# limix/CellRegMap

Measured on AMD Instinct MI355X. Metric: variant-tests/sec (interaction test), higher is better.
Workload: dtype f64

## Files before the change

cellregmap_amd/csrc/assemble.hip:

```cpp
#include "assemble.h"
#include "wave_ops.h"

namespace crm {

namespace {

__global__ __launch_bounds__(256) void woodbury_kernel(AssembleArgs a, const double* __restrict__ Gw, int KT,
                                                       double* __restrict__ Gext) {
    extern __shared__ double wsm[];
    const int k1 = a.wb_k1, KW = KT + k1, k0 = a.k0, c = a.c;
    const int b = blockIdx.x, tid = threadIdx.x;
    const NullFitOut fit = a.fit[b];
    const double g = fit.v0 * a.rho[fit.rho_index].rho;
    const double inv = 1.0 / fit.v1;
    const double* __restrict__ G = Gw + (long)b * KW * KW;
    double* __restrict__ out = Gext + (long)b * KT * KT;
    if (!(g > 0.0)) {
        for (int e = tid; e < KT * KT; e += 256) out[e] = G[(long)(e / KT) * KW + e % KT];
        return;
    }
    double* ME = wsm;
    double* Cm = ME + KT * k1;
    double* Z = Cm + k1 * k1;
    const long pos = a.sorted_pos[b];
    for (int e = tid; e < KT * k1; e += 256) {
        const int u = e / k1, f = e - u * k1;
        double plain;
        if (u < k0) plain = pos >= 0 ? a.wb_E1X[(long)f * a.wb_ldE1X + pos * k0 + u] : 0.0;
        else if (u < k0 + c) plain = a.wb_E1yW[(long)f * a.wb_ldE1yW + 1 + (u - k0)];
        else if (u == k0 + c) plain = a.wb_E1g[(long)f * a.wb_ldE1g + b];
        else plain = a.wb_E1yW[(long)f * a.wb_ldE1yW];
        ME[e] = (u < k0 && pos < 0) ? 0.0 : (plain - G[(long)u * KW + KT + f]) * inv;
    }
    for (int e = tid; e < k1 * k1; e += 256) {
        const int i = e / k1, j = e - i * k1;
        Cm[e] = (i == j ? 1.0 : 0.0) + g * (a.wb_EE[e] - G[(long)(KT + i) * KW + KT + j]) * inv;
    }
    __syncthreads();
    for (int j = 0; j < k1; j++) {
        if (tid == 0) Cm[j * k1 + j] = sqrt(Cm[j * k1 + j]);
        __syncthreads();
        const double l = Cm[j * k1 + j];
        for (int i = j + 1 + tid; i < k1; i += 256) Cm[i * k1 + j] /= l;
        __syncthreads();
        for (int e = tid; e < (k1 - j - 1) * (k1 - j - 1); e += 256) {
            const int i = j + 1 + e / (k1 - j - 1), q = j + 1 + e % (k1 - j - 1);
            if (q <= i) Cm[i * k1 + q] -= Cm[i * k1 + j] * Cm[q * k1 + j];
        }
        __syncthreads();
    }
    for (int u = tid; u < KT; u += 256) {
        for (int i = 0; i < k1; i++) {
            double s = ME[u * k1 + i];
            for (int q = 0; q < i; q++) s -= Cm[i * k1 + q] * Z[q * KT + u];
            Z[i * KT + u] = s / Cm[i * k1 + i];
        }
        for (int i = k1 - 1; i >= 0; i--) {
            double s = Z[i * KT + u];
            for (int q = i + 1; q < k1; q++) s -= Cm[q * k1 + i] * Z[q * KT + u];
            Z[i * KT + u] = s / Cm[i * k1 + i];
        }
    }
    __syncthreads();
    const double scale = fit.v1 * g;
    for (int e = tid; e < KT * KT; e += 256) {
        const int u = e / KT, v = e - u * KT;
        double s = 0.0;
        for (int f = 0; f < k1; f++) s += ME[u * k1 + f] * Z[f * KT + v];
        out[e] = G[(long)u * KW + v] + scale * s;
    }
}

__global__ __launch_bounds__(256) void woodbury_yty_kernel(AssembleArgs a, const double* __restrict__ Gw, int KT,
                                                           double* __restrict__ Gext) {
    extern __shared__ double wsm[];
    const int k1 = a.wb_k1, KW = KT + k1, k0 = a.k0, c = a.c;
    const int NR = k1 + KT, LD = NR | 1;
    const int b = blockIdx.x, tid = threadIdx.x;
    const int lane = tid & 63, wave = __builtin_amdgcn_readfirstlane(tid >> 6);
    const NullFitOut fit = a.fit[b];
    const double g = fit.v0 * a.rho[fit.rho_index].rho;
    const double inv = 1.0 / fit.v1;
    const double* __restrict__ G = Gw + (long)b * KW * KW;
    double* __restrict__ out = Gext + (long)b * KT * KT;
    if (!(g > 0.0)) {
        for (int e = tid; e < KT * KT; e += 256) out[e] = G[(long)(e / KT) * KW + e % KT];
        return;
    }
    double* AT = wsm;
    const long pos = a.sorted_pos[b];
    for (int e = tid; e < KT * k1; e += 256) {
        const int u = e / k1, f = e - u * k1;
        double plain;
        if (u < k0) plain = pos >= 0 ? a.wb_E1X[(long)f * a.wb_ldE1X + pos * k0 + u] : 0.0;
        else if (u < k0 + c) plain = a.wb_E1yW[(long)f * a.wb_ldE1yW + 1 + (u - k0)];
        else if (u == k0 + c) plain = a.wb_E1g[(long)f * a.wb_ldE1g + b];
        else plain = a.wb_E1yW[(long)f * a.wb_ldE1yW];
        AT[f * LD + k1 + u] = (u < k0 && pos < 0) ? 0.0 : (plain - G[(long)u * KW + KT + f]) * inv;
    }
    for (int e = tid; e < k1 * k1; e += 256) {
        const int i = e / k1, j = e - i * k1;
        if (j <= i) AT[j * LD + i] = (i == j ? 1.0 : 0.0) + g * (a.wb_EE[e] - G[(long)(KT + i) * KW + KT + j]) * inv;
    }
    __syncthreads();
    if (wave == 0) {
        const double l = sqrt(AT[0]);
        for (int R = lane; R < NR; R += 64) AT[R] = R == 0 ? l : AT[R] / l;
    }
    __syncthreads();
    for (int j = 0; j + 1 < k1; j++) {
        const double* colj = AT + j * LD;
        const double lnext = wave == 0 ? sqrt(fma(-colj[j + 1], colj[j + 1], AT[(j + 1) * LD + j + 1])) : 0.0;
        for (int R = ((j + 1) & ~63) + lane; R < NR; R += 64) {
            const double aR = R > j ? colj[R] : 0.0;
            for (int q0 = j + 1 + wave; q0 < k1; q0 += 16) {
                double lq[4], cv[4];
#pragma unroll
                for (int m = 0; m < 4; m++) {
                    const int q = q0 + 4 * m;
                    const bool on = q < k1 && R >= q;
                    lq[m] = on ? colj[q] : 0.0;
                    cv[m] = on ? AT[q * LD + R] : 0.0;
                }
#pragma unroll
                for (int m = 0; m < 4; m++) {
                    const int q = q0 + 4 * m;
                    if (!(q < k1 && R >= q)) continue;
                    double v = fma(-aR, lq[m], cv[m]);
                    if (q == j + 1) v = R == q ? lnext : v / lnext;
                    AT[q * LD + R] = v;
                }
            }
        }
        __syncthreads();
    }
    const int ts = (KT + 15) / 16, l15 = lane & 15, l4 = lane >> 4;
    const double scale = fit.v1 * g;
    const double* __restrict__ Y = AT + k1;
    int t = 0;
    for (int ti = 0; ti < ts; ti++)
        for (int tj = ti; tj < ts; tj++, t++) {
            if ((t & 3) != wave) continue;
            const int u = 16 * ti + l15, v = 16 * tj + l15;
            v4d acc = (v4d){0.0, 0.0, 0.0, 0.0};
            for (int f0 = 0; f0 < k1; f0 += 4) {
                const int f = f0 + l4;
                const double fa = (f < k1 && u < KT) ? Y[f * LD + u] : 0.0;
                const double fb = (f < k1 && v < KT) ? Y[f * LD + v] : 0.0;
                acc = __builtin_amdgcn_mfma_f64_16x16x4f64(fa, fb, acc, 0, 0, 0);
            }
#pragma unroll
            for (int reg = 0; reg < 4; reg++) {
                const int row = 16 * ti + l4 + 4 * reg;
                if (row < KT && v < KT && v >= row) {
                    const double s = scale * acc[reg];
                    out[(long)row * KT + v] = G[(long)row * KW + v] + s;
                    if (v != row) out[(long)v * KT + row] = G[(long)v * KW + row] + s;
                }
            }
        }
}

constexpr int PMAX = CRM_MAX_COV_XWIDE + 1;

__global__ __launch_bounds__(128) void finalize_kernel(AssembleArgs a, const double* __restrict__ Gext,
                                                        int KT, double* __restrict__ rows, int sym) {
    extern __shared__ double fsm[];
    __shared__ int ok_flag, keep_flag;
    __shared__ double rescale;
    const int Pd = a.c + 1;
    double* Lm = fsm;
    double* xky = Lm + Pd * Pd;
    double* uvec = xky + Pd;
    double* vv = uvec + a.k0;
    double* ww = vv + Pd;
    double* dkxm = rows ? rows + (size_t)blockIdx.x * 2 * a.k0 * Pd : ww + Pd;
    double* solm = dkxm + a.k0 * Pd;
#define L(i, j) Lm[(i) * Pd + (j)]
#define dkx(j, i) dkxm[(j) * Pd + (i)]
#define sol(j, i) solm[(j) * Pd + (i)]
    const int b = blockIdx.x;
    const NullFitOut fit = a.fit[b];
    const int k0 = a.k0, c = a.c;
    const int P = c + 1;
    const double v1 = fit.v1;
    const double inv = 1.0 / v1;
    const double* __restrict__ Ge = Gext + (long)b * KT * KT;
    const int tid = threadIdx.x;
    auto plain_xx = [&](int i, int j) -> double {
        if (i > j) { int t = i; i = j; j = t; }
        if (j < c) return a.WW[i * c + j];
        if (i < c) return a.gW[(long)b * a.ld_gW + i];
        return a.gg[b];
    };
    auto plain_xy = [&](int i) -> double { return i < c ? a.Wy[i] : a.gy[b]; };

    if (tid == 0) {
        bool ok = true;
        for (int i = 0; i < P; i++) {
            for (int j = 0; j <= i; j++)
                L(i, j) = (plain_xx(i, j) - Ge[(long)(k0 + i) * KT + (k0 + j)]) * inv;
            xky[i] = (plain_xy(i) - Ge[(long)(k0 + i) * KT + (k0 + c + 1)]) * inv;
        }
        bool keep = true;
        for (int j = 0; j < P && ok; j++) {
            double d = L(j, j);
            for (int k = 0; k < j; k++) d -= L(j, k) * L(j, k);
            if (!(d > 0.0)) {
                if (j == c) keep = false;
                else ok = false;
                break;
            }
            const double l = sqrt(d);
            L(j, j) = l;
            for (int i = j + 1; i < P; i++) {
                double s = L(i, j);
                for (int k = 0; k < j; k++) s -= L(i, k) * L(j, k);
                L(i, j) = s / l;
            }
        }
        if (ok && keep) {
            double nrm2 = 1.0;
            {
                for (int i = c - 1; i >= 0; i--) {
                    double sacc = L(c, i);
                    for (int k = i + 1; k < c; k++) sacc -= L(k, i) * vv[k];
                    vv[i] = sacc / L(i, i);
                }
                for (int j = 0; j < c; j++) {
                    const double t = vv[j] + (a.coef ? a.coef[(long)j * a.ld_coef + b] : 0.0);
                    nrm2 += t * t;
                }
            }
            const double lam_min = L(c, c) * L(c, c) / nrm2;
            for (int i = 0; i < P; i++) vv[i] = 1.0;
            double lam_max = 0.0;
            for (int it = 0; it < 12; it++) {
                const double vl = vv[c];
                for (int j = 0; j < c; j++) ww[j] = vv[j] + (a.coef ? a.coef[(long)j * a.ld_coef + b] : 0.0) * vl;
                ww[c] = vl;
                for (int i = 0; i < P; i++) {
                    double sacc = 0.0;
                    for (int k = i; k < P; k++) sacc += L(k, i) * ww[k];
                    vv[i] = sacc;
                }
                for (int i = P - 1; i >= 0; i--) {
                    double sacc = 0.0;
                    for (int k = 0; k <= i; k++) sacc += L(i, k) * vv[k];
                    ww[i] = sacc;
                }
                double last = ww[c];
                for (int j = 0; j < c; j++) last += (a.coef ? a.coef[(long)j * a.ld_coef + b] : 0.0) * ww[j];
                double n2 = last * last;
                for (int j = 0; j < c; j++) n2 += ww[j] * ww[j];
                lam_max = sqrt(n2);
                if (!(lam_max > 0.0)) break;
                for (int j = 0; j < c; j++) vv[j] = ww[j] / lam_max;
                vv[c] = last / lam_max;
            }
            if (lam_min <= 2.220446049250313e-16 * (double)P * lam_max) keep = false;
        }
        if (!keep) {
            for (int j = 0; j < c; j++) L(c, j) = 0.0;
            L(c, c) = 1.0;
            xky[c] = 0.0;
        }
        keep_flag = keep ? 1 : 0;
        rescale = 1.0;
        if (ok) {
            for (int i = 0; i < P; i++) {
                double s = xky[i];
                for (int k = 0; k < i; k++) s -= L(i, k) * xky[k];
                xky[i] = s / L(i, i);
            }
            if (fit.scale < 0.0) {
                double r = (a.yy - Ge[(long)(k0 + c + 1) * KT + (k0 + c + 1)]) * inv;
                const int used = c + ((fit.use_g && keep) ? 1 : 0);
                for (int i = 0; i < used; i++) r -= xky[i] * xky[i];
                const double df = (double)a.n - (double)(c + (fit.use_g ? 1 : 0));
                rescale = 1.0 / fmax(r / df, 1.4901161193847656e-08);
            }
            for (int i = P - 1; i >= 0; i--) {
                double s = xky[i];
                for (int k = i + 1; k < P; k++) s -= L(k, i) * xky[k];
                xky[i] = s / L(i, i);
            }
        }
        ok_flag = ok ? 1 : 0;
    }
    __syncthreads();
    const bool ok = ok_flag != 0;
    const bool keep_g = keep_flag != 0;
    for (int j = tid; j < k0; j += blockDim.x) {
        double row[PMAX];
        for (int i = 0; i < P; i++) {
            double plain;
            if (i < c) plain = a.Z1[(long)b * a.ldZ1 + (long)(1 + i) * k0 + j];
            else plain = a.Z2[(long)b * a.ldZ2 + j];
            double v = (plain - Ge[(long)j * KT + (k0 + i)]) * inv;
            if (i == c && !keep_g) v = 0.0;
            row[i] = v;
            dkx(j, i) = v;
        }
        for (int i = 0; i < P; i++) {
            double s = row[i];
            for (int k = 0; k < i; k++) s -= L(i, k) * row[k];
            row[i] = s / L(i, i);
        }
        for (int i = P - 1; i >= 0; i--) {
            double s = row[i];
            for (int k = i + 1; k < P; k++) s -= L(k, i) * row[k];
            row[i] = s / L(i, i);
        }
        for (int i = 0; i < P; i++) sol(j, i) = row[i];
        const double dky = (a.Z1[(long)b * a.ldZ1 + j] - Ge[(long)j * KT + (k0 + c + 1)]) * inv;
        double u = dky;
        for (int i = 0; i < P; i++) u -= dkx(j, i) * xky[i];
        uvec[j] = u * rescale;
    }
    __syncthreads();
    if (tid == 0) {
        double q = 0.0;
        for (int j = 0; j < k0; j++) q += uvec[j] * uvec[j];
        a.Q[b] = ok ? 0.5 * q : NAN;
    }
    double* __restrict__ F = a.F + (long)b * k0 * k0;
    for (int e = tid; e < k0 * k0; e += blockDim.x) {
        const int j = e / k0, jp = e - j * k0;
        const int lo = j < jp ? j : jp, hi = j < jp ? jp : j;
        const long pidx = (long)lo * k0 - (long)lo * (lo - 1) / 2 + (hi - lo);
        const int ja = sym ? lo : j, jb = sym ? hi : jp;
        double v = (a.Z3[(long)b * a.ldZ3 + pidx] - Ge[(long)ja * KT + jb]) * inv;
        for (int i = 0; i < P; i++) v -= dkx(ja, i) * sol(jb, i);
        F[e] = ok ? 0.5 * v * rescale : NAN;
    }
}
#undef L
#undef dkx
#undef sol

}

size_t woodbury_lds_bytes(int KT, int k1) { return sizeof(double) * ((size_t)2 * KT * k1 + (size_t)k1 * k1); }

size_t assemble_rows_scratch_doubles(int variants, int k0, int c) {
    const size_t P = (size_t)c + 1;
    const size_t lds = sizeof(double) * (P * P + 3 * P + k0 + 2 * (size_t)k0 * P);
    return lds > 150 * 1024 ? (size_t)variants * 2 * k0 * P : 0;
}

int launch_assemble(hipStream_t st, const AssembleArgs& a, int variants, double* Gext, double* fin_rows,
                    long* dma_launches) {
    if (variants <= 0) return CRM_OK;
    const int KT0 = a.k0 + a.c + 2;
    const int KT = KT0 + (a.wb_k1 > 0 ? a.wb_k1 : 0);
    double* const Gfin = Gext;
    if (a.wb_k1 > 0) {
        if (KT > CRM_MAX_GRAM_ROWS || woodbury_lds_bytes(KT0, a.wb_k1) > 150 * 1024 || !a.wb_Gw) {
            set_error("assemble: unrelated-donor form with %d + %d rows outside its supported range", KT0, a.wb_k1);
            return CRM_ERR_INTERNAL;
        }
        Gext = a.wb_Gw;
    }
    const int P = a.c + 1;
    const size_t fin_small = sizeof(double) * ((size_t)P * P + 3 * P + a.k0);
    size_t fin_lds = fin_small + sizeof(double) * 2 * (size_t)a.k0 * P;
    const bool rows_global = fin_lds > 150 * 1024;
    if (rows_global) fin_lds = fin_small;
    if (a.k0 > CRM_MAX_K0 || a.c > CRM_MAX_COV_XWIDE || KT > CRM_MAX_GRAM_ROWS || (rows_global && !fin_rows)) {
        set_error("assemble: k0=%d, c=%d outside the supported range (k0 <= %d, c <= %d, k0 + c + 2 <= %d)", a.k0, a.c,
                  CRM_MAX_K0, CRM_MAX_COV_XWIDE, CRM_MAX_GRAM_ROWS);
        return CRM_ERR_UNSUPPORTED;
    }
    const bool gram_done = a.wb_k1 > 0 && a.wb_gram_done != 0;
    bool dma = gram_done;
    if (!gram_done) CRM_TRY(launch_gram_ext(st, a, variants, Gext, KT, &dma));
    if (dma && dma_launches) ++*dma_launches;
    const bool yty = a.wb_k1 > 0 && form("woodbury_ytY", 1) != 0;
    if (a.wb_k1 > 0) {
        const size_t lds = yty ? sizeof(double) * a.wb_k1 * (size_t)((KT0 + a.wb_k1) | 1) : woodbury_lds_bytes(KT0, a.wb_k1);
        CRM_HIP(yty ? launch_with_lds(woodbury_yty_kernel, dim3(variants), dim3(256), lds, st, lds > 60 * 1024, a, a.wb_Gw, KT0, Gfin)
                    : launch_with_lds(woodbury_kernel, dim3(variants), dim3(256), lds, st, lds > 60 * 1024, a, a.wb_Gw, KT0, Gfin));
    }
    CRM_HIP(launch_with_lds(finalize_kernel, dim3(variants), dim3(128), fin_lds, st, fin_lds > 60 * 1024, a, Gfin, KT0,
                            rows_global ? fin_rows : nullptr, yty ? 1 : 0));
    return CRM_OK;
}

}
```

Measured before the change: 85530.

## Add single-wave row-oriented Cholesky path to Woodbury ytY kernel

```diff
diff --git a/cellregmap_amd/csrc/assemble.hip b/cellregmap_amd/csrc/assemble.hip
--- a/cellregmap_amd/csrc/assemble.hip
+++ b/cellregmap_amd/csrc/assemble.hip
@@ -71,6 +71,17 @@
     }
 }
 
+constexpr int CB = 4;
+
+__device__ __forceinline__ void rows_take_left(double (&v)[CB], const double* own, const double* lq, int LD, int q0) {
+    for (int j = 0; j < q0; j++) {
+        const double aj = own[j * LD];
+#pragma unroll
+        for (int m = 0; m < CB; m++) v[m] = fma(-aj, lq[j * LD + m], v[m]);
+    }
+}
+
+template <int ROWS>
 __global__ __launch_bounds__(256) void woodbury_yty_kernel(AssembleArgs a, const double* __restrict__ Gw, int KT,
                                                            double* __restrict__ Gext) {
     extern __shared__ double wsm[];
@@ -89,50 +100,135 @@
     }
     double* AT = wsm;
     const long pos = a.sorted_pos[b];
-    for (int e = tid; e < KT * k1; e += 256) {
-        const int u = e / k1, f = e - u * k1;
-        double plain;
-        if (u < k0) plain = pos >= 0 ? a.wb_E1X[(long)f * a.wb_ldE1X + pos * k0 + u] : 0.0;
-        else if (u < k0 + c) plain = a.wb_E1yW[(long)f * a.wb_ldE1yW + 1 + (u - k0)];
-        else if (u == k0 + c) plain = a.wb_E1g[(long)f * a.wb_ldE1g + b];
-        else plain = a.wb_E1yW[(long)f * a.wb_ldE1yW];
-        AT[f * LD + k1 + u] = (u < k0 && pos < 0) ? 0.0 : (plain - G[(long)u * KW + KT + f]) * inv;
-    }
-    for (int e = tid; e < k1 * k1; e += 256) {
-        const int i = e / k1, j = e - i * k1;
-        if (j <= i) AT[j * LD + i] = (i == j ? 1.0 : 0.0) + g * (a.wb_EE[e] - G[(long)(KT + i) * KW + KT + j]) * inv;
+    if (ROWS) {
+        constexpr int LB = 4;
+        for (int e0 = tid; e0 < KT * k1; e0 += 256 * LB) {
+            double plain[LB], gw[LB];
+#pragma unroll
+            for (int m = 0; m < LB; m++) {
+                const int e = min(e0 + 256 * m, KT * k1 - 1), u = e / k1, f = e - u * k1;
+                const double* yW = a.wb_E1yW + (long)f * a.wb_ldE1yW;
+                const double* p = u < k0 ? (pos >= 0 ? a.wb_E1X + (long)f * a.wb_ldE1X + pos * k0 + u : yW)
+                                : u < k0 + c ? yW + 1 + (u - k0)
+                                : u == k0 + c ? a.wb_E1g + (long)f * a.wb_ldE1g + b : yW;
+                plain[m] = *p;
+                gw[m] = G[(long)u * KW + KT + f];
+            }
+#pragma unroll
+            for (int m = 0; m < LB; m++) {
+                const int e = e0 + 256 * m, u = e / k1, f = e - u * k1;
+                if (e < KT * k1) AT[f * LD + k1 + u] = (u < k0 && pos < 0) ? 0.0 : (plain[m] - gw[m]) * inv;
+            }
+        }
+        for (int e0 = tid; e0 < k1 * k1; e0 += 256 * LB) {
+            double ee[LB], gw[LB];
+#pragma unroll
+            for (int m = 0; m < LB; m++) {
+                const int e = min(e0 + 256 * m, k1 * k1 - 1), i = e / k1, j = e - i * k1;
+                ee[m] = a.wb_EE[e];
+                gw[m] = G[(long)(KT + i) * KW + KT + j];
+            }
+#pragma unroll
+            for (int m = 0; m < LB; m++) {
+                const int e = e0 + 256 * m, i = e / k1, j = e - i * k1;
+                if (e < k1 * k1) AT[j * LD + i] = j <= i ? (i == j ? 1.0 : 0.0) + g * (ee[m] - gw[m]) * inv : 0.0;
+            }
+        }
+    } else {
+        for (int e = tid; e < KT * k1; e += 256) {
+            const int u = e / k1, f = e - u * k1;
+            double plain;
+            if (u < k0) plain = pos >= 0 ? a.wb_E1X[(long)f * a.wb_ldE1X + pos * k0 + u] : 0.0;
+            else if (u < k0 + c) plain = a.wb_E1yW[(long)f * a.wb_ldE1yW + 1 + (u - k0)];
+            else if (u == k0 + c) plain = a.wb_E1g[(long)f * a.wb_ldE1g + b];
+            else plain = a.wb_E1yW[(long)f * a.wb_ldE1yW];
+            AT[f * LD + k1 + u] = (u < k0 && pos < 0) ? 0.0 : (plain - G[(long)u * KW + KT + f]) * inv;
+        }
+        for (int e = tid; e < k1 * k1; e += 256) {
+            const int i = e / k1, j = e - i * k1;
+            if (j <= i) AT[j * LD + i] = (i == j ? 1.0 : 0.0) + g * (a.wb_EE[e] - G[(long)(KT + i) * KW + KT + j]) * inv;
+        }
     }
     __syncthreads();
-    if (wave == 0) {
-        const double l = sqrt(AT[0]);
-        for (int R = lane; R < NR; R += 64) AT[R] = R == 0 ? l : AT[R] / l;
-    }
-    __syncthreads();
-    for (int j = 0; j + 1 < k1; j++) {
-        const double* colj = AT + j * LD;
-        const double lnext = wave == 0 ? sqrt(fma(-colj[j + 1], colj[j + 1], AT[(j + 1) * LD + j + 1])) : 0.0;
-        for (int R = ((j + 1) & ~63) + lane; R < NR; R += 64) {
-            const double aR = R > j ? colj[R] : 0.0;
-            for (int q0 = j + 1 + wave; q0 < k1; q0 += 16) {
-                double lq[4], cv[4];
-#pragma unroll
-                for (int m = 0; m < 4; m++) {
-                    const int q = q0 + 4 * m;
-                    const bool on = q < k1 && R >= q;
-                    lq[m] = on ? colj[q] : 0.0;
-                    cv[m] = on ? AT[q * LD + R] : 0.0;
-                }
-#pragma unroll
-                for (int m = 0; m < 4; m++) {
-                    const int q = q0 + 4 * m;
-                    if (!(q < k1 && R >= q)) continue;
-                    double v = fma(-aR, lq[m], cv[m]);
-                    if (q == j + 1) v = R == q ? lnext : v / lnext;
-                    AT[q * LD + R] = v;
-                }
-            }
-        }
-        __syncthreads();
+    if (ROWS) {
+        if (wave == 0) {
+            const int R = lane < k1 ? lane : k1 - 1;
+            const double* own = AT + R;
+            for (int q0 = 0; q0 < k1; q0 += CB) {
+                double v[CB];
+#pragma unroll
+                for (int m = 0; m < CB; m++) v[m] = q0 + m < k1 ? AT[(q0 + m) * LD + R] : 0.0;
+                rows_take_left(v, own, AT + q0, LD, q0);
+#pragma unroll
+                for (int m = 0; m < CB; m++) {
+                    const int q = q0 + m;
+                    if (q >= k1) break;
+                    const double l = sqrt(read_lane(v[m], q));
+                    const double y = R == q ? l : v[m] / l;
+                    if (lane >= q && lane < k1) AT[q * LD + lane] = y;
+#pragma unroll
+                    for (int m2 = m + 1; m2 < CB; m2++)
+                        v[m2] = fma(-y, read_lane(y, q0 + m2 < k1 ? q0 + m2 : q), v[m2]);
+                }
+                __builtin_amdgcn_fence(__ATOMIC_RELEASE, "wavefront");
+                __builtin_amdgcn_wave_barrier();
+                __builtin_amdgcn_fence(__ATOMIC_ACQUIRE, "wavefront");
+            }
+        }
+        __syncthreads();
+        const int per = (KT + 3) / 4, u = wave * per + lane;
+        if (lane < per && u < KT) {
+            double* own = AT + k1 + u;
+            for (int q0 = 0; q0 < k1; q0 += CB) {
+                double v[CB];
+#pragma unroll
+                for (int m = 0; m < CB; m++) v[m] = q0 + m < k1 ? own[(q0 + m) * LD] : 0.0;
+                rows_take_left(v, own, AT + q0, LD, q0);
+#pragma unroll
+                for (int m = 0; m < CB; m++) {
+                    const int q = q0 + m;
+                    if (q >= k1) break;
+                    const double* colq = AT + q * LD;
+                    const double y = v[m] / colq[q];
+                    own[q * LD] = y;
+#pragma unroll
+                    for (int m2 = m + 1; m2 < CB; m2++) v[m2] = fma(-y, colq[q0 + m2], v[m2]);
+                }
+            }
+        }
+        __syncthreads();
+    } else {
+        if (wave == 0) {
+            const double l = sqrt(AT[0]);
+            for (int R = lane; R < NR; R += 64) AT[R] = R == 0 ? l : AT[R] / l;
+        }
+        __syncthreads();
+        for (int j = 0; j + 1 < k1; j++) {
+            const double* colj = AT + j * LD;
+            const double lnext = wave == 0 ? sqrt(fma(-colj[j + 1], colj[j + 1], AT[(j + 1) * LD + j + 1])) : 0.0;
+            for (int R = ((j + 1) & ~63) + lane; R < NR; R += 64) {
+                const double aR = R > j ? colj[R] : 0.0;
+                for (int q0 = j + 1 + wave; q0 < k1; q0 += 16) {
+                    double lq[4], cv[4];
+#pragma unroll
+                    for (int m = 0; m < 4; m++) {
+                        const int q = q0 + 4 * m;
+                        const bool on = q < k1 && R >= q;
+                        lq[m] = on ? colj[q] : 0.0;
+                        cv[m] = on ? AT[q * LD + R] : 0.0;
+                    }
+#pragma unroll
+                    for (int m = 0; m < 4; m++) {
+                        const int q = q0 + 4 * m;
+                        if (!(q < k1 && R >= q)) continue;
+                        double v = fma(-aR, lq[m], cv[m]);
+                        if (q == j + 1) v = R == q ? lnext : v / lnext;
+                        AT[q * LD + R] = v;
+                    }
+                }
+            }
+            __syncthreads();
+        }
     }
     const int ts = (KT + 15) / 16, l15 = lane & 15, l4 = lane >> 4;
     const double scale = fit.v1 * g;
@@ -142,6 +238,14 @@
         for (int tj = ti; tj < ts; tj++, t++) {
             if ((t & 3) != wave) continue;
             const int u = 16 * ti + l15, v = 16 * tj + l15;
+            double gv[4], gm[4];
+#pragma unroll
+            for (int reg = 0; reg < 4; reg++) {
+                const int row = 16 * ti + l4 + 4 * reg;
+                const bool on = ROWS && row < KT && v < KT && v >= row;
+                gv[reg] = on ? G[(long)row * KW + v] : 0.0;
+                gm[reg] = on && v != row ? G[(long)v * KW + row] : 0.0;
+            }
             v4d acc = (v4d){0.0, 0.0, 0.0, 0.0};
             for (int f0 = 0; f0 < k1; f0 += 4) {
                 const int f = f0 + l4;
@@ -154,8 +258,8 @@
                 const int row = 16 * ti + l4 + 4 * reg;
                 if (row < KT && v < KT && v >= row) {
                     const double s = scale * acc[reg];
-                    out[(long)row * KT + v] = G[(long)row * KW + v] + s;
-                    if (v != row) out[(long)v * KT + row] = G[(long)v * KW + row] + s;
+                    out[(long)row * KT + v] = (ROWS ? gv[reg] : G[(long)row * KW + v]) + s;
+                    if (v != row) out[(long)v * KT + row] = (ROWS ? gm[reg] : G[(long)v * KW + row]) + s;
                 }
             }
         }
@@ -376,11 +480,14 @@
     bool dma = gram_done;
     if (!gram_done) CRM_TRY(launch_gram_ext(st, a, variants, Gext, KT, &dma));
     if (dma && dma_launches) ++*dma_launches;
-    const bool yty = a.wb_k1 > 0 && form("woodbury_ytY", 1) != 0;
+    const int wb_form = a.wb_k1 > 0 ? form("woodbury_ytY", 2) : 0;
+    const bool yty = wb_form != 0;
     if (a.wb_k1 > 0) {
+        const bool rows = wb_form != 1 && a.wb_k1 <= 64;
         const size_t lds = yty ? sizeof(double) * a.wb_k1 * (size_t)((KT0 + a.wb_k1) | 1) : woodbury_lds_bytes(KT0, a.wb_k1);
-        CRM_HIP(yty ? launch_with_lds(woodbury_yty_kernel, dim3(variants), dim3(256), lds, st, lds > 60 * 1024, a, a.wb_Gw, KT0, Gfin)
-                    : launch_with_lds(woodbury_kernel, dim3(variants), dim3(256), lds, st, lds > 60 * 1024, a, a.wb_Gw, KT0, Gfin));
+        CRM_HIP(!yty   ? launch_with_lds(woodbury_kernel, dim3(variants), dim3(256), lds, st, lds > 60 * 1024, a, a.wb_Gw, KT0, Gfin)
+                : rows ? launch_with_lds(woodbury_yty_kernel<1>, dim3(variants), dim3(256), lds, st, lds > 60 * 1024, a, a.wb_Gw, KT0, Gfin)
+                       : launch_with_lds(woodbury_yty_kernel<0>, dim3(variants), dim3(256), lds, st, lds > 60 * 1024, a, a.wb_Gw, KT0, Gfin));
     }
     CRM_HIP(launch_with_lds(finalize_kernel, dim3(variants), dim3(128), fin_lds, st, fin_lds > 60 * 1024, a, Gfin, KT0,
                             rows_global ? fin_rows : nullptr, yty ? 1 : 0));
```

Result: no change. 86310, median of 6 (+0.9%).
